# gillet-thomas/NeuroViT

Hardware: AMD Instinct MI355X
Metric: fMRI volumes/sec (fwd+bwd) ViT3D 128^3 p16 d768 L12 [timed step = fwd+bwd+AdamW update] (higher is better)
Workload: dtype bf16; 1 GPU; ViT3D-base 128^3 patch 16, train step (fwd+bwd+AdamW), batch 4/GPU, dropout 0; global_batch=4, parallelism=dp1, grad_buckets=7, grad_allreduce=none (1 GPU)

## Files before the change

### include/neurovit_hip.h

```cpp
#ifndef NEUROVIT_HIP_H
#define NEUROVIT_HIP_H

#ifdef __cplusplus
extern "C" {
#endif

#define NV_OK 0
#define NV_ERR_ARG (-1)
#define NV_ERR_HIP (-2)
#define NV_ERR_ARCH (-3)

int nv_version(void);
int nv_arch_ok(void);
const char* nv_last_error(void);

#define NV_OPERAND_BF16 0
#define NV_OPERAND_FP16 1
int nv_set_operand_format(int fmt);
int nv_operand_format(void);

int nv_prof_enable(int on);
int nv_prof_summary(int kind, double* ms, double* work, long* count);
int nv_prof_summary_bytes(int kind, double* bytes);

// ... 42 lines not shown
  int keep_grads;
  float* params; float* grads; float* adam_m; float* adam_v; void* params16;
} nv_adamw_arena;
int nv_gemm_bf16_grouped_adamw(int count, const nv_gemm_problem* problems, const nv_adamw_arena* opt, void* stream);
int nv_adamw_ranges(const nv_adamw_arena* opt, const long* begins, const long* lens, int count, void* stream);

int nv_gemm_set_tile(int bm, int bn);

int nv_gemm_lnfold_supported(int M, int N, int K);
long nv_ln_fold_stats_floats(int M, int d);
int nv_ln_fold_weight(const float* W, long ldw, int N, int K, const float* gamma, const float* beta, const float* bias, void* Wg16, long ldg,
                      float* colsum, float* fbias, void* stream);
int nv_gemm_resid_ln(int M, int N, int K, const void* A, long lda, const void* W, long ldw, const float* bias, const float* resid, long ldr, float* out,
                     long ldo, void* out16, long ldo16, float* stats, void* stream);
int nv_gemm_lnfold(int gelu, int M, int N, int K, const void* X16, long ldx, const void* Wg16, long ldw, const float* stats, const float* colsum,
                   const float* fbias, float eps, void* out16, long ldo, void* stream);

int nv_skinny_nt(int epi, int R, int N, int K, const void* A, long lda, const void* W, long ldw, const float* bias, const float* resid,
                 long ldr, void* out, long ldo, void* u_out, long ldu, unsigned long drop_seed, float drop_p, void* stream);
int nv_skinny_nn(int epi, int R, int N, int K, const void* A, long lda, const void* W, long ldw, const void* u, long ldu, void* out, long ldo,
                 float* dcol, int accumulate, unsigned long drop_seed, float drop_p, void* stream);
int nv_skinny_nn_sparse(int R, int N, int K, const void* A, long lda, const void* W, long ldw, void* out, long total_rows, int keep_every,
                        void* stream);

int nv_ln_fwd(const float* x, long ldx, int M, int d, const float* gamma, const float* beta, float eps, void* y, long ldy,
              float* mean, float* rstd, void* stream);
long nv_ln_bwd_workspace_bytes(int M, int d);
int nv_ln_bwd(const float* dy, long lddy, const float* x, long ldx, const float* mean, const float* rstd, const float* gamma,
              int M, int d, const float* g_in, float* g_out, long ldg, void* g16, long ldg16, float* dgamma, float* dbeta,
              float* dcolsum, int accumulate, void* workspace, long ws_bytes, unsigned long drop_seed, float drop_p,
              void* stream, void* reduce_stream);
#define NV_LN_NO_REDUCE ((void*)(-1L))
int nv_ln_bwd_reduce(const void* workspace, int M, int d, float* dgamma, float* dbeta, float* dcolsum, int accumulate, void* stream);

typedef struct nv_reduce_job {
  const float* partials;
  int rows, width, nseg;
  float* out[3];
  int accumulate;
} nv_reduce_job;
int nv_reduce_multi(const nv_reduce_job* jobs, int count, void* stream);
int nv_ln_bwd_partial_rows(int M);

long nv_zscore_crop_workspace_bytes(int B);
int nv_volume_sigma(const void* raw, int dtype, const long* strides5, int B, const int* crop8, float eps, float* sigma, float* mean,
                    void* workspace, long ws_bytes, void* stream);
// ... 353 lines not shown
```

### neurovit_amd/_cabi.py

```python
from __future__ import annotations

import ctypes
import os
import re
from typing import Dict, List, Tuple

_HERE = os.path.dirname(os.path.abspath(__file__))
HEADER = os.path.join(os.path.dirname(_HERE), "include", "neurovit_hip.h")
LIB_PATH = os.environ.get("NEUROVIT_HIP_LIB") or os.path.join(_HERE, "lib", "libneurovit_hip.so")

_SCALARS = {"int": ctypes.c_int, "long": ctypes.c_long, "float": ctypes.c_float, "double": ctypes.c_double}


class VitConfig(ctypes.Structure):
    _fields_ = [("image_size", ctypes.c_int), ("image_patch_size", ctypes.c_int), ("frames", ctypes.c_int),
                ("frame_patch_size", ctypes.c_int), ("channels", ctypes.c_int), ("num_classes", ctypes.c_int),
                ("dim", ctypes.c_int), ("depth", ctypes.c_int), ("heads", ctypes.c_int), ("dim_head", ctypes.c_int),
                ("mlp_dim", ctypes.c_int), ("ln_eps", ctypes.c_float), ("pool_mean", ctypes.c_int),
                ("image_width", ctypes.c_int), ("patch_width", ctypes.c_int),
                ("no_proj_dropout", ctypes.c_int)]


class VitInput(ctypes.Structure):
    _fields_ = [("vol_sigma", ctypes.c_void_p), ("time_points", ctypes.c_int), ("rows_form", ctypes.c_int), ("attn_export", ctypes.c_void_p)]
# ... 85 lines not shown
        if self._dll is None:
            if not os.path.exists(LIB_PATH):
                raise RuntimeError(
                    f"neurovit_amd: {LIB_PATH} not found - build it with `python -c 'import __graft_entry__ as g; g.build()'` "
                    "(or `make -C neurovit_amd/csrc`). There is no CPU / PyTorch fallback for this path.")
            dll = ctypes.CDLL(LIB_PATH)
            for name, (restype, argtypes) in self.protos.items():
                fn = getattr(dll, name)
                fn.restype, fn.argtypes = restype, argtypes
            got = dll.nv_abi_version()
            if got != ABI_VERSION:
                raise RuntimeError(f"neurovit_amd: {LIB_PATH} has ABI revision {got}, this binding expects {ABI_VERSION} - rebuild the library "
                                   "(make -C neurovit_amd/csrc); see INTEGRATION.md 'ABI revisions'")
            if os.environ.get("NEUROVIT_ATTN_MODE"):
                dll.nv_attn_set_mode(int(os.environ["NEUROVIT_ATTN_MODE"]))
            if os.environ.get("NEUROVIT_ADAMW_WGS"):
                dll.nv_gemm_set_tile(12, int(os.environ["NEUROVIT_ADAMW_WGS"]))
            if os.environ.get("NEUROVIT_HEAD_STEP"):
                dll.nv_vit_set_head_step(int(os.environ["NEUROVIT_HEAD_STEP"]))
            if os.environ.get("NEUROVIT_WGRAD_WGS"):
                dll.nv_gemm_set_tile(14, int(os.environ["NEUROVIT_WGRAD_WGS"]))
            if os.environ.get("NEUROVIT_PATCH_MODE"):
                dll.nv_patch_set_mode(int(os.environ["NEUROVIT_PATCH_MODE"]))
            if os.environ.get("NEUROVIT_ADAMW_CAP"):
                dll.nv_gemm_set_tile(13, int(os.environ["NEUROVIT_ADAMW_CAP"]))
            self._dll = dll
        return self._dll

    def __getattr__(self, name):
        return getattr(self.load(), name)


lib = _Lib()


OPERAND_FORMATS = {"bf16": 0, "fp16": 1}
_operand_format = "bf16"


def set_operand_format(fmt: str) -> None:
    global _operand_format
    if fmt != _operand_format:
        if fmt not in OPERAND_FORMATS:
            raise ValueError(f"neurovit_amd: operand format must be 'bf16' or 'fp16', got {fmt!r}")
        check(lib.nv_set_operand_format(OPERAND_FORMATS[fmt]), "nv_set_operand_format")
        _operand_format = fmt
# ... 23 lines not shown
```

### neurovit_amd/csrc/engine.hip

```cpp
#include <stdlib.h>
#include <string.h>

#include <unordered_map>
#include <utility>
#include <vector>

#include "../../include/neurovit_hip.h"

#include "common.h"

namespace {

inline long align_up(long v, long a) { return (v + a - 1) / a * a; }

struct Dims {
  int B, N, n, P, Ppad, d, inner, m, L, C, heads, dh, M, T;
  int gf, gh, gw;
  int pool_mean;
};

static int g_cls_tail = 1;
extern "C" int nv_vit_set_cls_tail(int on) { g_cls_tail = on ? 1 : 0; return 0; }
static int g_head_step = 1;
extern "C" int nv_vit_set_head_step(int on) { g_head_step = on ? 1 : 0; return 0; }
// ... 591 lines not shown
    RUN(nv_attn_fwd(ws + w.qkv, 3 * D.inner, B, D.n, D.heads, D.dh, scale, ws + w.ao, D.inner, (float*)(ws + w.lse), site_seed(drop_seed, 4 * l + 0), drop_p, stream));
    if (tail && l == D.L - 1) {
      RUN(cls_rows_block16(D, q, w, l, p, p16, ws, eps, xin, x1, x2, st2, ws + w.u, drop_seed, drop_p, proj_drop_p(cfg, drop_p), stream));
      xin = x2;
      continue;
    }
    RUN(nv_gemm_bf16(0, 4, M, d, D.inner, ws + w.ao, D.inner, p16 + q.wo, D.inner, x1, d, p + q.bo, xin, d, nullptr, 0, 0, 1.f, site_seed(drop_seed, 4 * l + 1), proj_drop_p(cfg, drop_p), stream));
    RUN(nv_ln_fwd_f8_train(x1, d, M, d, p + q.n2g, p + q.n2b, eps, s_xn2, x8, d, ws + w.xn2, d, st2, st2 + M, stream));
    RUN(nv_gemm_f8_gelu_train(M, D.m, d, x8, d, p8 + q.w1, d, cs + 3L * D.inner, p + q.b1, s_h, h8, D.m, ws + w.h, D.m, ws + w.u, D.m,
                              site_seed(drop_seed, 4 * l + 2), drop_p, stream));
    RUN(nv_gemm_f8_resid_drop(M, d, D.m, h8, D.m, p8 + q.w2, D.m, x2, d, cs + 3L * D.inner + D.m, p + q.b2, x1, d, site_seed(drop_seed, 4 * l + 3), drop_p, stream));
    xin = x2;
  }
  return pool_head(D, T, p, eps, xin, ws, W.xm, W.xh, W.hst, logits, stream);
}

namespace {

struct BwdCall {
  const float* video; const long* strides5; const float* params; const void* params16; void* workspace; long ws_bytes; const float* dlogits;
  float* grads; void* grads16;
  int accumulate, first_stage, last_stage; float drop_p, emb_drop_p; unsigned long drop_seed; void* stream; void* aux_stream; int join_aux, rows_form;
  const nv_adamw_arena* fuse; int fuse_mode;
  const nv_vit_backward_opts* opts;
  const nv_vit_attn_grad_export* attn_grad;
};

struct BwdLayer { int l; bool tail; int Mr; long rs; };

struct Bwd {
  const nv_vit_config* cfg; const BwdCall& c; const Dims& D; const ParamTab& T; const WS& W;
  char* ws; const float* p; const r16* p16; float* g;
  bool wg, tail_fwd;
  int M, d, acc, du_tile_rows;
  float scale;
  hipStream_t S, A;
  float* GR(long off) const { return c.grads ? c.grads + off : nullptr; }
  void* M16(long off) const { return c.grads16 ? (void*)((r16*)c.grads16 + off) : nullptr; }
  float* dxn1(int l) const { return (float*)(ws + (l == D.L - 1 ? W.hookg : W.dxn)); }

  int bwd_head() const {
    const float* xlast = (float*)(ws + W.layer[D.L - 1].x2);
    return nv_head_bwd(c.dlogits, D.B, D.C, p + T.hw, D.pool_mean ? (const float*)(ws + W.xm) : xlast, D.pool_mean ? (long)d : (long)D.n * d,
                       (float*)(ws + W.hst), (float*)(ws + W.xh), p + T.hg, d, D.n, g, d, ws + W.scratch(D.L - 1).g16, d,
                       GR(T.hg), GR(T.hb), GR(T.hw), GR(T.hbias), GR(T.layer[D.L - 1].b2), acc, ws + W.sc[0].red, W.red_bytes,
                       site_seed(c.drop_seed, 4 * (D.L - 1) + 3), c.drop_p, D.pool_mean, S);
  }

  int bwd_ffn(const BwdLayer& R) const {
// ... 67 lines not shown
    }
    RUN(nv_reduce_multi(jobs, nj, A));
    nv_gemm_problem pr[4];
    pr[0] = {d, D.m, Mr, g16, d * rs, ws + w.h, D.m * rs, GR(q.w2), D.m, acc, M16(q.w2), D.m};
    pr[1] = {D.m, d, Mr, du, D.m * rs, ws + w.xn2, d * rs, GR(q.w1), d, acc, M16(q.w1), d};
    pr[2] = {d, D.inner, Mr, g16b, d * rs, ws + w.ao, D.inner * rs, GR(q.wo), D.inner, acc, M16(q.wo), D.inner};
    pr[3] = {3 * D.inner, d, M, dqkv, 3 * D.inner, ws + w.xn1, d, GR(q.wqkv), d, acc, M16(q.wqkv), d};
    if (c.fuse && c.fuse_mode != 3) return nv_gemm_bf16_grouped_adamw(4, pr, c.fuse, A);
    return nv_gemm_bf16_grouped(2, 1, 4, pr, A);
  }

  int bwd_embed_tokens() const {
    float* est = (float*)(ws + W.est);
    return nv_embed_finish_bwd(g, d, (float*)(ws + W.t), d, est, est + D.T, p + T.pe_g2, D.B, D.N, d, (float*)(ws + W.dt), d, ws + W.dt16, d, GR(T.pe_g2),
                               GR(T.pe_b2), GR(T.pe_bias), GR(T.pos), GR(T.cls), acc, ws + W.sc[1].red, W.red_bytes, site_seed(c.drop_seed, 4 * D.L), c.emb_drop_p, S);
  }

  int bwd_embed() const {
    float* pst = (float*)(ws + W.pst);
    float* const dvideo = c.opts ? c.opts->dvideo : nullptr;
    const void* wpe = (D.P != D.Ppad) ? (const void*)(ws + W.wpe16) : (const void*)(p16 + T.pe_w);
    void* redA = ws + (A != S ? W.sc[0].red2 : W.sc[0].red);
    const long redA_bytes = A != S ? W.red2_bytes : W.red_bytes;
    RUN(nv_gemm_bf16(1, 1, D.T, D.Ppad, d, ws + W.dt16, d, wpe, D.Ppad, ws + W.dxp, D.Ppad, nullptr, nullptr, 0, nullptr, 0, 0, 1.f, 0, 0.f, A));
    if (dvideo)
      RUN(nv_patch_ln_dx(c.video, c.strides5, D.B, cfg->channels, cfg->frames, cfg->image_size, img_w(cfg), cfg->image_patch_size, pat_w(cfg), cfg->frame_patch_size,
                         (const float*)(ws + W.dxp), D.Ppad, pst, pst + D.T, p + T.pe_g, dvideo, c.opts->dvideo_strides5, A));
    if (!wg) return NV_OK;
    RUN(nv_patch_ln_bwd(c.video, c.strides5, D.B, cfg->channels, cfg->frames, cfg->image_size, img_w(cfg), cfg->image_patch_size,
                        pat_w(cfg), cfg->frame_patch_size, (float*)(ws + W.dxp), D.Ppad, pst, pst + D.T, GR(T.pe_g), GR(T.pe_b), acc, redA, redA_bytes, A));
    if (D.P != D.Ppad) {
      RUN(nv_gemm_bf16(2, 1, d, D.Ppad, D.T, ws + W.dt16, d, ws + W.xp, D.Ppad, ws + W.dwpe, D.Ppad, nullptr, nullptr, 0, nullptr, 0, 0, 1.f, 0, 0.f, S));
      return nv_copy_2d_f32((float*)(ws + W.dwpe), D.Ppad, d, D.P, GR(T.pe_w), D.P, acc, S);
    }
    return nv_gemm_bf16(2, 1, d, D.P, D.T, ws + W.dt16, d, ws + W.xp, D.Ppad, GR(T.pe_w), D.P, nullptr, nullptr, 0, M16(T.pe_w), D.P, acc, 1.f, 0, 0.f, S);
  }
};

}

static int backward_impl(const Layout& Y, const nv_vit_config* cfg, const BwdCall& c) {
  const Dims& D = Y.D; const WS& W = Y.W;
  const nv_adamw_arena* fuse = c.fuse; const nv_vit_backward_opts* opts = c.opts;
  NV_CHECK_ARG(!fuse || (!c.accumulate && !c.grads16 && fuse->grads == c.grads && c.first_stage <= 1 && c.last_stage == D.L + 1),
               "nv_vit_backward: the optimizer update during the backward pass needs accumulate = 0, no bf16 mirror, its own gradient arena and every stage in one call");
  const bool wg = !opts || opts->weight_grads;
  NV_CHECK_ARG(!fuse || !opts, "nv_vit_backward: the optimizer update during the backward pass takes no input gradient / data-only options");
  NV_CHECK_ARG(!fuse || !c.attn_grad, "nv_vit_backward: the optimizer update during the backward pass exports no attention gradients");
  NV_CHECK_ARG(!opts || !opts->dvideo || opts->dvideo_strides5, "nv_vit_backward_ex: dvideo needs dvideo_strides5");
  NV_CHECK_ARG(wg || (!c.grads && !c.grads16), "nv_vit_backward_ex: the data-only backward (weight_grads = 0) writes no gradient arena - pass grads = grads16 = NULL");
  NV_CHECK_ARG(c.video && c.strides5 && c.params && c.params16 && c.workspace && c.dlogits && (c.grads || !wg), "nv_vit_backward: null pointer");
  NV_CHECK_ARG(c.ws_bytes >= W.total, "nv_vit_backward: workspace too small (%ld < %ld) - forward must run with training=1", c.ws_bytes, W.total);
  NV_CHECK_ARG(nv_aligned16(c.grads) && nv_aligned16(c.grads16), "nv_vit_backward: grads / grads16 must be 16-byte aligned");
  NV_CHECK_ARG(c.first_stage >= 0 && c.last_stage <= D.L + 1 && c.first_stage <= c.last_stage, "nv_vit_backward_stages: bad stage range [%d, %d]", c.first_stage, c.last_stage);
  hipStream_t S = (hipStream_t)c.stream;
  hipStream_t A = (c.aux_stream && wg) ? (hipStream_t)c.aux_stream : S;
  const bool forked = (A != S);
  char* ws = (char*)c.workspace;
// ... 240 lines not shown
  const Dims& D = Y.D; const ParamTab& T = Y.T; const WS& W = Y.W;
  RUN(forward_in_impl(Y, cfg, B, video, shape5, strides5, in, params, params16, workspace, ws_bytes, 1, drop_p, emb_drop_p, drop_seed, logits, stream, head_fused));
  if (head_fused) {
    char* ws = (char*)workspace;
    const int Ll = D.L - 1;
    RUN(nv_head_step_soft((const float*)(ws + W.layer[Ll].x2), (long)D.n * D.d, B, D.d, params + T.hg, params + T.hb, cfg->ln_eps, params + T.hw, params + T.hbias, D.C,
                          labels, lscale, hp->loss_scale_state, lo, (float*)(ws + W.xh), (float*)(ws + W.hst), logits, loss, dlogits, D.n, (float*)(ws + W.g), D.d,
                          ws + W.scratch(Ll).g16, D.d, grads + T.hg, grads + T.hb, grads + T.hw, grads + T.hbias, grads + T.layer[Ll].b2,
                          hp->accumulate ? 1 : 0, ws + W.sc[0].red, W.red_bytes, site_seed(drop_seed, 4 * Ll + 3), drop_p, stream));
  } else {
    RUN(nv_ce_loss_soft(logits, labels, B, cfg->num_classes, lscale, hp->loss_scale_state, lo, loss, dlogits, stream));
  }
  nv_adamw_arena opt;
  opt.struct_size = (int)sizeof(opt); opt.step = hp->step; opt.lr = hp->lr; opt.beta1 = hp->beta1; opt.beta2 = hp->beta2; opt.eps = hp->eps;
  opt.weight_decay = hp->weight_decay; opt.grad_scale = hp->grad_scale / lscale; opt.keep_grads = hp->fuse_update == 2;
  opt.params = params; opt.grads = grads; opt.adam_m = adam_m; opt.adam_v = adam_v; opt.params16 = params16;
  BwdCall bc{};
  bc.video = video; bc.strides5 = strides5; bc.params = params; bc.params16 = params16; bc.workspace = workspace; bc.ws_bytes = ws_bytes;
  bc.dlogits = dlogits; bc.grads = grads; bc.accumulate = hp->accumulate ? 1 : 0; bc.drop_p = drop_p; bc.emb_drop_p = emb_drop_p; bc.drop_seed = drop_seed;
  bc.stream = stream; bc.aux_stream = aux_stream; bc.join_aux = 1; bc.rows_form = in ? in->rows_form : 0;
  if (dp && hp->update) return dp_backward_update(Y, cfg, bc, params, params16, adam_m, adam_v, hp, dp, head_fused, lscale);
  bc.first_stage = head_fused ? 1 : 0; bc.last_stage = cfg->depth + 1;
  bc.fuse = fused ? &opt : nullptr; bc.fuse_mode = hp->fuse_update;
  RUN(backward_impl(Y, cfg, bc));
  if (hp->update && !fused) {
    RUN(final_update(hp, params, params16, grads, nullptr, adam_m, adam_v, T.total, hp->grad_scale / lscale, stream));
  } else if (fused) {
    std::vector<long> begins, lens;
    long cur = 0;
    auto skip = [&](long off, long numel) { if (off > cur) { begins.push_back(cur); lens.push_back(off - cur); } cur = align_up(off + numel, 8); };
    for (int l = 0; l < D.L; ++l) {
      const LinearW lw = linear_weights(D, T.layer[l]);
      for (int i = 0; i < 4; ++i) skip(lw.off[i], lw.numel[i]);
    }
    if (T.total > cur) { begins.push_back(cur); lens.push_back(T.total - cur); }
    RUN(nv_adamw_ranges(&opt, begins.data(), lens.data(), (int)begins.size(), stream));
  }
  return NV_OK;
}
```

### neurovit_amd/csrc/norm.hip

```cpp
#include "common.h"

#define WAVES_PER_BLOCK 4

#include <type_traits>
template <typename OT>
__device__ __forceinline__ void store4(OT* p, const f32x4& o) {
  if constexpr (std::is_same<OT, float>::value) *reinterpret_cast<f32x4*>(p) = o;
  else *reinterpret_cast<r16x4*>(p) = cvt4<OT>(o[0], o[1], o[2], o[3]);
}
__device__ __forceinline__ r16 cvt1_rt(float v, int fp16) { return fp16 ? cvt1<fp16_t>(v) : cvt1<bf16_t>(v); }

template <int NV>
__device__ __forceinline__ void row_load(const float* row, int d, int lane, f32x4 (&x)[NV]) {
#pragma unroll
  for (int v = 0; v < NV; ++v) {
    const int c = (lane + 64 * v) * 4;
    x[v] = (c < d) ? *reinterpret_cast<const f32x4*>(row + c) : f32x4{0.f, 0.f, 0.f, 0.f};
  }
}
template <int NV>
__device__ __forceinline__ void row_stats(const f32x4 (&x)[NV], int d, int lane, float eps, float& mean, float& rstd) {
  float s = 0.f;
#pragma unroll
  for (int v = 0; v < NV; ++v) s += (x[v][0] + x[v][1]) + (x[v][2] + x[v][3]);
// ... 902 lines not shown
                                   unsigned long drop_seed, float drop_p, void* stream) {
  const DropCfg drop = make_drop(drop_seed, drop_p);
  NV_CHECK_ARG(B > 0 && N > 0 && (d % 4) == 0 && d <= 2048, "nv_embed_finish_fwd: d=%d must be a multiple of 4 and <= 2048", d);
  NV_CHECK_ARG((ldt % 4) == 0 && (ldx % 4) == 0, "nv_embed_finish_fwd: leading dims must be multiples of 4");
  const int rows = B * (N + 1);
  const dim3 grid((rows + WAVES_PER_BLOCK - 1) / WAVES_PER_BLOCK), block(256);
  hipStream_t s = (hipStream_t)stream;
  if (d <= 1024) hipLaunchKernelGGL(embed_finish_fwd_kernel<4>, grid, block, 0, s, t, ldt, B, N, d, gamma, beta, eps, pos, cls, x, ldx, mean, rstd, drop);
  else hipLaunchKernelGGL(embed_finish_fwd_kernel<8>, grid, block, 0, s, t, ldt, B, N, d, gamma, beta, eps, pos, cls, x, ldx, mean, rstd, drop);
  NV_CHECK_LAUNCH("nv_embed_finish_fwd");
  return NV_OK;
}

__global__ void batch_sum_kernel(const float* __restrict__ g, long ldg, int B, int n, int d, float* dpos, float* dcls, int accumulate) {
  const long idx = (long)blockIdx.x * blockDim.x + threadIdx.x;
  if (idx >= (long)n * d) return;
  const int i = (int)(idx / d), c = (int)(idx - (long)i * d);
  float s = 0.f;
  for (int b = 0; b < B; ++b) s += g[((long)b * n + i) * ldg + c];
  if (dpos) dpos[idx] = accumulate ? dpos[idx] + s : s;
  if (i == 0 && dcls) dcls[c] = accumulate ? dcls[c] + s : s;
}

__global__ void apply_drop_kernel(float* __restrict__ g, long count, DropCfg drop) {
  const long i = ((long)blockIdx.x * blockDim.x + threadIdx.x) * 4;
  if (i >= count) return;
  f32x4 v = *reinterpret_cast<f32x4*>(g + i);
  v *= drop_factor4(drop, (unsigned long long)i);
  *reinterpret_cast<f32x4*>(g + i) = v;
}

extern "C" long nv_embed_finish_bwd_workspace_bytes(int B, int N, int d) { return nv_ln_bwd_workspace_bytes(B * N, d); }

extern "C" int nv_embed_finish_bwd(const float* g, long ldg, const float* t, long ldt, const float* mean, const float* rstd,
                                   const float* gamma, int B, int N, int d, float* dt, long lddt, void* dt16, long lddt16,
                                   float* dgamma, float* dbeta, float* dbias_pe, float* dpos, float* dcls, int accumulate,
                                   void* workspace, long ws_bytes, unsigned long drop_seed, float drop_p, void* stream) {
  hipStream_t s = (hipStream_t)stream;
  const DropCfg drop = make_drop(drop_seed, drop_p);
  if (drop.thresh) {
    NV_CHECK_ARG(ldg == d, "nv_embed_finish_bwd: dropout needs a dense g");
    const long count = (long)B * (N + 1) * d;
    hipLaunchKernelGGL(apply_drop_kernel, dim3((unsigned)((count / 4 + 255) / 256)), dim3(256), 0, s, (float*)g, count, drop);
    NV_CHECK_LAUNCH("nv_embed_finish_bwd/drop");
  }
  NV_CHECK_ARG(B > 0 && N > 0 && (d % 4) == 0 && d <= 2048, "nv_embed_finish_bwd: bad dims");
  const int n = N + 1;
  const long need = nv_embed_finish_bwd_workspace_bytes(B, N, d);
  NV_CHECK_ARG(ws_bytes >= need, "nv_embed_finish_bwd: workspace too small");
  const bool params_out = dgamma || dbeta || dbias_pe || dpos || dcls;
  NV_CHECK_ARG(!params_out || (dgamma && dbeta && dbias_pe && dpos && dcls), "nv_embed_finish_bwd: the parameter gradients are all given or all NULL");
  {
    const int rc = ln_bwd_launch(g + ldg, ldg, t, ldt, mean, rstd, gamma, B * N, d, nullptr, dt, lddt, dt16, lddt16, dgamma, dbeta, dbias_pe,
                                 accumulate, workspace, ws_bytes, 0, 0.f, stream, params_out ? nullptr : NV_LN_NO_REDUCE, N, 1);
    if (rc) return rc;
  }
  if (!params_out) return NV_OK;
  const long tot = (long)n * d;
  hipLaunchKernelGGL(batch_sum_kernel, dim3((unsigned)((tot + 255) / 256)), dim3(256), 0, s, g, ldg, B, n, d, dpos, dcls, accumulate);
  NV_CHECK_LAUNCH("nv_embed_finish_bwd/batch_sum");
  return NV_OK;
}

__device__ __forceinline__ void head_fwd_row(int b, float* sh, const float* __restrict__ x, long row_stride, int d, const float* __restrict__ gamma,
                                             const float* __restrict__ beta, float eps, const float* __restrict__ Wt,
                                             const float* __restrict__ bias, int C, float* __restrict__ xh_out,
                                             float* __restrict__ stats_out, float* __restrict__ logits) {
  float* xs = sh;
  float* scratch = sh + d;
  const int tid = threadIdx.x, lane = tid & 63, wid = tid >> 6;
  const float* row = x + (long)b * row_stride;
  float s = 0.f;
  for (int c = tid; c < d; c += 256) { xs[c] = row[c]; s += xs[c]; }
  s = wave_sum(s);
  if (lane == 0) scratch[wid] = s;
  __syncthreads();
  const float mean = ((scratch[0] + scratch[1]) + (scratch[2] + scratch[3])) / (float)d;
  float q = 0.f;
  for (int c = tid; c < d; c += 256) { const float t = xs[c] - mean; q += t * t; }
  q = wave_sum(q);
  if (lane == 0) scratch[4 + wid] = q;
  __syncthreads();
// ... 336 lines not shown
```

### neurovit_amd/csrc/skinny.hip

```cpp
#include "common.h"

namespace {

constexpr int SK_R = 4;

enum { SK_NT_RESID = 0, SK_NT_GELU = 1 };
enum { SK_NN_DGELU = 0, SK_NN_F32 = 1, SK_NN_BF16 = 2 };

template <int EPI, typename T>
__global__ __launch_bounds__(256) void skinny_nt_kernel(const r16* __restrict__ A, long lda, int R, const r16* __restrict__ W, long ldw, int N, int K,
                                                        const float* __restrict__ bias, const float* __restrict__ resid, long ldr,
                                                        void* __restrict__ out, long ldo, r16* __restrict__ u_out, long ldu, DropCfg drop) {
  const int lane = threadIdx.x & 63, n = blockIdx.x * 4 + (threadIdx.x >> 6);
  const int r0 = blockIdx.y * SK_R, rows = (R - r0 < SK_R) ? R - r0 : SK_R;
  if (n >= N) return;
  float acc[SK_R];
#pragma unroll
  for (int r = 0; r < SK_R; ++r) acc[r] = 0.f;
  const r16* w = W + (long)n * ldw;
  for (int k = lane * 8; k < K; k += 4 * 512) {
    r16x8 wq[4], aq[4][SK_R];
#pragma unroll
    for (int q = 0; q < 4; ++q) {
      const int kq = k + 512 * q;
// ... 44 lines not shown
template <int EPI, typename T>
__global__ __launch_bounds__(1024) void skinny_nn_kernel(const r16* __restrict__ A, long lda, int R, const r16* __restrict__ W, long ldw, int N, int K,
                                                         const r16* __restrict__ u, long ldu, void* __restrict__ out, long ldo,
                                                         float* __restrict__ dcol, int accumulate, long fill_rows, int keep_every, DropCfg drop) {
  extern __shared__ __attribute__((aligned(16))) float sk_lds[];
  if (blockIdx.z == 1) {
    zero_rows_except(reinterpret_cast<char*>(out), fill_rows, (long)N * 2, keep_every, blockIdx.y * gridDim.x + blockIdx.x, gridDim.x * gridDim.y);
    return;
  }
  float (*part)[NN_KK][SK_R][NN_COLS] = reinterpret_cast<float (*)[NN_KK][SK_R][NN_COLS]>(sk_lds);
  float (*red)[SK_R][NN_COLS] = reinterpret_cast<float (*)[SK_R][NN_COLS]>(sk_lds + 16 * NN_KK * SK_R * NN_COLS);
  const int tid = threadIdx.x, lane = tid & 63, wv = tid >> 6, ng = lane & (NN_COLS / 8 - 1), kk = lane / (NN_COLS / 8);
  const int n0 = blockIdx.x * NN_COLS, nc = n0 + ng * 8;
  const int r0 = blockIdx.y * SK_R, rows = (R - r0 < SK_R) ? R - r0 : SK_R;
  float acc[SK_R][8];
#pragma unroll
  for (int r = 0; r < SK_R; ++r)
#pragma unroll
    for (int e = 0; e < 8; ++e) acc[r][e] = 0.f;
  if (nc < N) {
    constexpr int STEP = 16 * NN_KK;
    for (int k = wv * NN_KK + kk; k < K; k += 4 * STEP) {
      r16x8 wq[4];
      float aq[4][SK_R];
#pragma unroll
      for (int q = 0; q < 4; ++q) {
        const int kq = k + STEP * q;
        if (kq < K) {
          wq[q] = *reinterpret_cast<const r16x8*>(W + (long)kq * ldw + nc);
#pragma unroll
          for (int r = 0; r < SK_R; ++r)
            if (r < rows) aq[q][r] = dec1<T>(A[(long)(r0 + r) * lda + kq]);
        }
      }
#pragma unroll
      for (int q = 0; q < 4; ++q) {
        if (k + STEP * q < K) {
#pragma unroll
          for (int r = 0; r < SK_R; ++r) {
            if (r < rows) {
#pragma unroll
              for (int e = 0; e < 8; ++e) acc[r][e] = __builtin_fmaf(aq[q][r], dec1<T>(wq[q][e]), acc[r][e]);
            }
          }
        }
      }
    }
  }
#pragma unroll
  for (int r = 0; r < SK_R; ++r) {
    *reinterpret_cast<f32x4*>(&part[wv][kk][r][ng * 8]) = f32x4{acc[r][0], acc[r][1], acc[r][2], acc[r][3]};
    *reinterpret_cast<f32x4*>(&part[wv][kk][r][ng * 8 + 4]) = f32x4{acc[r][4], acc[r][5], acc[r][6], acc[r][7]};
  }
  __syncthreads();
  {
    const int w = tid / (SK_R * NN_COLS), rc = tid % (SK_R * NN_COLS);
    float v = 0.f;
#pragma unroll
    for (int q = 0; q < NN_KK; ++q) v += part[w][q][rc / NN_COLS][rc % NN_COLS];
    red[w][rc / NN_COLS][rc % NN_COLS] = v;
  }
  __syncthreads();
  const int c = tid % NN_COLS, r = tid / NN_COLS;
  float stored = 0.f;
  const bool live = r < rows && n0 + c < N;
// ... 8 lines not shown
      const r16 o = cvt1<T>(v * keep * gelu_grad_f(dec1<T>(u[row * ldu + n])));
      ((r16*)out)[row * ldo + n] = o;
      stored = dec1<T>(o);
    } else if constexpr (EPI == SK_NN_F32) {
      ((float*)out)[row * ldo + n] = v;
    } else {
      ((r16*)out)[row * ldo + n] = cvt1<T>(v);
    }
  }
  if constexpr (EPI == SK_NN_DGELU) {
    if (dcol) {
      __syncthreads();
      if (r < SK_R) red[0][r][c] = live ? stored : 0.f;
      __syncthreads();
      if (r == 0 && n0 + c < N) {
        float s = 0.f;
#pragma unroll
        for (int q = 0; q < SK_R; ++q) s += red[0][q][c];
        dcol[n0 + c] = (accumulate ? dcol[n0 + c] : 0.f) + s;
      }
    }
  }
}

constexpr int NN_LDS = (16 * NN_KK * SK_R * NN_COLS + 16 * SK_R * NN_COLS) * (int)sizeof(float);
template <typename T>
void nn_attrs_fmt() {
  (void)hipFuncSetAttribute(reinterpret_cast<const void*>(skinny_nn_kernel<SK_NN_DGELU, T>), hipFuncAttributeMaxDynamicSharedMemorySize, NN_LDS);
  (void)hipFuncSetAttribute(reinterpret_cast<const void*>(skinny_nn_kernel<SK_NN_F32, T>), hipFuncAttributeMaxDynamicSharedMemorySize, NN_LDS);
  (void)hipFuncSetAttribute(reinterpret_cast<const void*>(skinny_nn_kernel<SK_NN_BF16, T>), hipFuncAttributeMaxDynamicSharedMemorySize, NN_LDS);
}
void nn_attrs() {
  static bool attr = false;
  if (attr) return;
  nn_attrs_fmt<bf16_t>(); nn_attrs_fmt<fp16_t>();
  attr = true;
}

}

extern "C" int nv_skinny_nt(int epi, int R, int N, int K, const void* A, long lda, const void* W, long ldw, const float* bias, const float* resid,
                            long ldr, void* out, long ldo, void* u_out, long ldu, unsigned long drop_seed, float drop_p, void* stream) {
  NV_CHECK_ARG(drop_p == 0.f || (ldo % N) == 0, "nv_skinny_nt: with dropout `out` must be a row-strided view of a dense [M, N] tensor (ldo a multiple of N)");
  const DropCfg drop = make_drop(drop_seed, drop_p);
  NV_CHECK_ARG(R > 0 && N > 0 && K > 0 && (K % 8) == 0 && (lda % 8) == 0 && (ldw % 8) == 0 && A && W && bias && out && nv_aligned16(A) && nv_aligned16(W),
               "nv_skinny_nt: K, lda, ldw must be multiples of 8, operands 16-byte aligned");
  NV_CHECK_ARG(epi == SK_NT_GELU || (epi == SK_NT_RESID && resid), "nv_skinny_nt: epilogue 0 needs resid; epilogues are 0 (bias + residual, f32) and 1 (bias + GELU, bf16)");
  const dim3 grid((N + 3) / 4, (R + SK_R - 1) / SK_R), block(256);
  hipStream_t s = (hipStream_t)stream;
  NV_DISPATCH_OPERAND(T,
    if (epi == SK_NT_RESID)
      hipLaunchKernelGGL((skinny_nt_kernel<SK_NT_RESID, T>), grid, block, 0, s, (const r16*)A, lda, R, (const r16*)W, ldw, N, K, bias, resid, ldr, out, ldo, (r16*)nullptr, 0L, drop);
    else
      hipLaunchKernelGGL((skinny_nt_kernel<SK_NT_GELU, T>), grid, block, 0, s, (const r16*)A, lda, R, (const r16*)W, ldw, N, K, bias, resid, ldr, out, ldo, (r16*)u_out, ldu, drop));
  NV_CHECK_LAUNCH("nv_skinny_nt");
  return NV_OK;
}

extern "C" int nv_skinny_nn(int epi, int R, int N, int K, const void* A, long lda, const void* W, long ldw, const void* u, long ldu, void* out, long ldo,
                            float* dcol, int accumulate, unsigned long drop_seed, float drop_p, void* stream) {
  NV_CHECK_ARG(drop_p == 0.f || (epi == SK_NN_DGELU && (ldo % N) == 0), "nv_skinny_nn: dropout only with epilogue 0, `out` a row-strided view of a dense [M, N] tensor");
  const DropCfg drop = make_drop(drop_seed, drop_p);
  NV_CHECK_ARG(R > 0 && N > 0 && K > 0 && (N % 8) == 0 && (ldw % 8) == 0 && A && W && out && nv_aligned16(W), "nv_skinny_nn: N, ldw must be multiples of 8, W 16-byte aligned");
  NV_CHECK_ARG(epi >= 0 && epi <= 2 && (epi != SK_NN_DGELU || u) && (!dcol || (epi == SK_NN_DGELU && R <= SK_R)), "nv_skinny_nn: epilogue 0 needs u; column sums only with epilogue 0 and R <= 4");
  const dim3 grid((N + NN_COLS - 1) / NN_COLS, (R + SK_R - 1) / SK_R), block(1024);
  hipStream_t s = (hipStream_t)stream;
  nn_attrs();
#define SK_NN(E) hipLaunchKernelGGL((skinny_nn_kernel<E, T>), grid, block, NN_LDS, s, (const r16*)A, lda, R, (const r16*)W, ldw, N, K, (const r16*)u, ldu, out, ldo, dcol, accumulate, 0L, 0, drop)
  NV_DISPATCH_OPERAND(T, if (epi == SK_NN_DGELU) SK_NN(SK_NN_DGELU); else if (epi == SK_NN_F32) SK_NN(SK_NN_F32); else SK_NN(SK_NN_BF16));
#undef SK_NN
  NV_CHECK_LAUNCH("nv_skinny_nn");
  return NV_OK;
}

extern "C" int nv_skinny_nn_sparse(int R, int N, int K, const void* A, long lda, const void* W, long ldw, void* out, long total_rows, int keep_every,
                                   void* stream) {
  NV_CHECK_ARG(R > 0 && N > 0 && K > 0 && (N % 8) == 0 && (ldw % 8) == 0 && A && W && out && nv_aligned16(W) && nv_aligned16(out) && keep_every >= 1 &&
                   (long)(R - 1) * keep_every < total_rows && (long)R * keep_every >= total_rows,
               "nv_skinny_nn_sparse: N, ldw multiples of 8; W, out 16-byte aligned; R = ceil(total_rows / keep_every) (every kept row is computed: the fill skips them all)");
  const dim3 grid((N + NN_COLS - 1) / NN_COLS, (R + SK_R - 1) / SK_R, 2), block(1024);
  nn_attrs();
  NV_DISPATCH_OPERAND(T, hipLaunchKernelGGL((skinny_nn_kernel<SK_NN_BF16, T>), grid, block, NN_LDS, (hipStream_t)stream, (const r16*)A, lda, R, (const r16*)W, ldw, N, K,
                                            (const r16*)nullptr, 0L, out, (long)N * keep_every, (float*)nullptr, 0, total_rows, keep_every, make_drop(0, 0.f)));
  NV_CHECK_LAUNCH("nv_skinny_nn_sparse");
  return NV_OK;
}
```

Measured before the change: 1191 volumes/s.

## Add split-K skinny NN kernel, vectorized batch sum, and overlap rest-param AdamW

Adds a split-K variant of the skinny NN GEMM. When K exceeds 2048 by default, it spreads the reduction over many workgroups and merges the partial sums through a global scratch buffer with an atomic last-block counter, so that only a few row tiles no longer underfill the GPU. It also vectorizes the position/cls gradient batch-sum to float4 with one block per token. Separately, when fused updates are on and an aux stream exists, it splits the remaining-parameter AdamW update across two streams and moves the patch-embed dx GEMM to the main stream. The existing skinny NN inner loop now loads A values as bf16 and clamps out-of-range k instead of branching. The split-K path relies on device-global counters and scratch, which adds a cross-block synchronisation risk.

```diff
diff --git a/include/neurovit_hip.h b/include/neurovit_hip.h
--- a/include/neurovit_hip.h
+++ b/include/neurovit_hip.h
@@ -88,6 +88,7 @@
                  float* dcol, int accumulate, unsigned long drop_seed, float drop_p, void* stream);
 int nv_skinny_nn_sparse(int R, int N, int K, const void* A, long lda, const void* W, long ldw, void* out, long total_rows, int keep_every,
                         void* stream);
+int nv_skinny_set_mode(int mode);
 
 int nv_ln_fwd(const float* x, long ldx, int M, int d, const float* gamma, const float* beta, float eps, void* y, long ldy,
               float* mean, float* rstd, void* stream);
diff --git a/neurovit_amd/_cabi.py b/neurovit_amd/_cabi.py
--- a/neurovit_amd/_cabi.py
+++ b/neurovit_amd/_cabi.py
@@ -131,6 +131,8 @@
                 dll.nv_gemm_set_tile(14, int(os.environ["NEUROVIT_WGRAD_WGS"]))
             if os.environ.get("NEUROVIT_PATCH_MODE"):
                 dll.nv_patch_set_mode(int(os.environ["NEUROVIT_PATCH_MODE"]))
+            if os.environ.get("NEUROVIT_SKINNY_MODE"):
+                dll.nv_skinny_set_mode(int(os.environ["NEUROVIT_SKINNY_MODE"]))
             if os.environ.get("NEUROVIT_ADAMW_CAP"):
                 dll.nv_gemm_set_tile(13, int(os.environ["NEUROVIT_ADAMW_CAP"]))
             self._dll = dll
diff --git a/neurovit_amd/csrc/engine.hip b/neurovit_amd/csrc/engine.hip
--- a/neurovit_amd/csrc/engine.hip
+++ b/neurovit_amd/csrc/engine.hip
@@ -637,9 +637,33 @@
   float* grads; void* grads16;
   int accumulate, first_stage, last_stage; float drop_p, emb_drop_p; unsigned long drop_seed; void* stream; void* aux_stream; int join_aux, rows_form;
   const nv_adamw_arena* fuse; int fuse_mode;
+  bool fuse_rest;
   const nv_vit_backward_opts* opts;
   const nv_vit_attn_grad_export* attn_grad;
 };
+
+void rest_update_ranges(const Dims& D, const ParamTab& T, int part, std::vector<long>& begins, std::vector<long>& lens) {
+  const long main_iv[3][2] = {{T.pos, T.pe_g}, {T.pe_w, T.layer[0].n1g}, {T.layer[D.L - 1].b2, T.total}};
+  auto push = [&](long b, long e) { if (e > b) { begins.push_back(b); lens.push_back(e - b); } };
+  auto emit = [&](long b, long e) {
+    if (part == 0) return push(b, e);
+    for (int i = 0; i < 3 && b < e; ++i) {
+      const long lo = main_iv[i][0], hi = main_iv[i][1];
+      if (hi <= b || lo >= e) continue;
+      if (lo > b) { if (part == 2) push(b, lo); b = lo; }
+      const long m = hi < e ? hi : e;
+      if (part == 1) push(b, m);
+      b = m;
+    }
+    if (part == 2) push(b, e);
+  };
+  long cur = 0;
+  for (int l = 0; l < D.L; ++l) {
+    const LinearW lw = linear_weights(D, T.layer[l]);
+    for (int i = 0; i < 4; ++i) { emit(cur, lw.off[i]); cur = align_up(lw.off[i] + lw.numel[i], 8); }
+  }
+  emit(cur, T.total);
+}
 
 struct BwdLayer { int l; bool tail; int Mr; long rs; };
 
@@ -753,7 +777,9 @@
     const void* wpe = (D.P != D.Ppad) ? (const void*)(ws + W.wpe16) : (const void*)(p16 + T.pe_w);
     void* redA = ws + (A != S ? W.sc[0].red2 : W.sc[0].red);
     const long redA_bytes = A != S ? W.red2_bytes : W.red_bytes;
-    RUN(nv_gemm_bf16(1, 1, D.T, D.Ppad, d, ws + W.dt16, d, wpe, D.Ppad, ws + W.dxp, D.Ppad, nullptr, nullptr, 0, nullptr, 0, 0, 1.f, 0, 0.f, A));
+    const hipStream_t Q = c.fuse_rest ? S : A;
+    RUN(nv_gemm_bf16(1, 1, D.T, D.Ppad, d, ws + W.dt16, d, wpe, D.Ppad, ws + W.dxp, D.Ppad, nullptr, nullptr, 0, nullptr, 0, 0, 1.f, 0, 0.f, Q));
+    if (c.fuse_rest) RUN(stream_sync(S, A));
     if (dvideo)
       RUN(nv_patch_ln_dx(c.video, c.strides5, D.B, cfg->channels, cfg->frames, cfg->image_size, img_w(cfg), cfg->image_patch_size, pat_w(cfg), cfg->frame_patch_size,
                          (const float*)(ws + W.dxp), D.Ppad, pst, pst + D.T, p + T.pe_g, dvideo, c.opts->dvideo_strides5, A));
@@ -762,9 +788,17 @@
                         pat_w(cfg), cfg->frame_patch_size, (float*)(ws + W.dxp), D.Ppad, pst, pst + D.T, GR(T.pe_g), GR(T.pe_b), acc, redA, redA_bytes, A));
     if (D.P != D.Ppad) {
       RUN(nv_gemm_bf16(2, 1, d, D.Ppad, D.T, ws + W.dt16, d, ws + W.xp, D.Ppad, ws + W.dwpe, D.Ppad, nullptr, nullptr, 0, nullptr, 0, 0, 1.f, 0, 0.f, S));
-      return nv_copy_2d_f32((float*)(ws + W.dwpe), D.Ppad, d, D.P, GR(T.pe_w), D.P, acc, S);
-    }
-    return nv_gemm_bf16(2, 1, d, D.P, D.T, ws + W.dt16, d, ws + W.xp, D.Ppad, GR(T.pe_w), D.P, nullptr, nullptr, 0, M16(T.pe_w), D.P, acc, 1.f, 0, 0.f, S);
+      RUN(nv_copy_2d_f32((float*)(ws + W.dwpe), D.Ppad, d, D.P, GR(T.pe_w), D.P, acc, S));
+    } else {
+      RUN(nv_gemm_bf16(2, 1, d, D.P, D.T, ws + W.dt16, d, ws + W.xp, D.Ppad, GR(T.pe_w), D.P, nullptr, nullptr, 0, M16(T.pe_w), D.P, acc, 1.f, 0, 0.f, S));
+    }
+    if (!c.fuse_rest) return NV_OK;
+    std::vector<long> b, n;
+    rest_update_ranges(D, T, 1, b, n);
+    RUN(nv_adamw_ranges(c.fuse, b.data(), n.data(), (int)b.size(), S));
+    b.clear(); n.clear();
+    rest_update_ranges(D, T, 2, b, n);
+    return nv_adamw_ranges(c.fuse, b.data(), n.data(), (int)b.size(), A);
   }
 };
 
@@ -1051,18 +1085,13 @@
   if (dp && hp->update) return dp_backward_update(Y, cfg, bc, params, params16, adam_m, adam_v, hp, dp, head_fused, lscale);
   bc.first_stage = head_fused ? 1 : 0; bc.last_stage = cfg->depth + 1;
   bc.fuse = fused ? &opt : nullptr; bc.fuse_mode = hp->fuse_update;
+  bc.fuse_rest = fused && aux_stream && aux_stream != stream;
   RUN(backward_impl(Y, cfg, bc));
   if (hp->update && !fused) {
     RUN(final_update(hp, params, params16, grads, nullptr, adam_m, adam_v, T.total, hp->grad_scale / lscale, stream));
-  } else if (fused) {
+  } else if (fused && !bc.fuse_rest) {
     std::vector<long> begins, lens;
-    long cur = 0;
-    auto skip = [&](long off, long numel) { if (off > cur) { begins.push_back(cur); lens.push_back(off - cur); } cur = align_up(off + numel, 8); };
-    for (int l = 0; l < D.L; ++l) {
-      const LinearW lw = linear_weights(D, T.layer[l]);
-      for (int i = 0; i < 4; ++i) skip(lw.off[i], lw.numel[i]);
-    }
-    if (T.total > cur) { begins.push_back(cur); lens.push_back(T.total - cur); }
+    rest_update_ranges(D, T, 0, begins, lens);
     RUN(nv_adamw_ranges(&opt, begins.data(), lens.data(), (int)begins.size(), stream));
   }
   return NV_OK;
diff --git a/neurovit_amd/csrc/norm.hip b/neurovit_amd/csrc/norm.hip
--- a/neurovit_amd/csrc/norm.hip
+++ b/neurovit_amd/csrc/norm.hip
@@ -948,6 +948,32 @@
   if (i == 0 && dcls) dcls[c] = accumulate ? dcls[c] + s : s;
 }
 
+__global__ __launch_bounds__(256) void batch_sum4_kernel(const float* __restrict__ g, long ldg, int B, int n, int d, float* dpos, float* dcls, int accumulate) {
+  const int i = blockIdx.x;
+  for (int c = threadIdx.x * 4; c < d; c += 256 * 4) {
+    const float* src = g + (long)i * ldg + c;
+    const long bstep = (long)n * ldg;
+    f32x4 s = {0.f, 0.f, 0.f, 0.f};
+    int b = 0;
+    for (; b + 4 <= B; b += 4) {
+      f32x4 v[4];
+#pragma unroll
+      for (int q = 0; q < 4; ++q) v[q] = *reinterpret_cast<const f32x4*>(src + (b + q) * bstep);
+#pragma unroll
+      for (int q = 0; q < 4; ++q) s += v[q];
+    }
+    for (; b < B; ++b) s += *reinterpret_cast<const f32x4*>(src + b * bstep);
+    if (dpos) {
+      f32x4* o = reinterpret_cast<f32x4*>(dpos + (long)i * d + c);
+      *o = accumulate ? *o + s : s;
+    }
+    if (i == 0 && dcls) {
+      f32x4* o = reinterpret_cast<f32x4*>(dcls + c);
+      *o = accumulate ? *o + s : s;
+    }
+  }
+}
+
 __global__ void apply_drop_kernel(float* __restrict__ g, long count, DropCfg drop) {
   const long i = ((long)blockIdx.x * blockDim.x + threadIdx.x) * 4;
   if (i >= count) return;
@@ -983,7 +1009,10 @@
   }
   if (!params_out) return NV_OK;
   const long tot = (long)n * d;
-  hipLaunchKernelGGL(batch_sum_kernel, dim3((unsigned)((tot + 255) / 256)), dim3(256), 0, s, g, ldg, B, n, d, dpos, dcls, accumulate);
+  if ((ldg % 4) == 0 && nv_aligned16(g) && nv_aligned16(dpos) && nv_aligned16(dcls))
+    hipLaunchKernelGGL(batch_sum4_kernel, dim3((unsigned)n), dim3(256), 0, s, g, ldg, B, n, d, dpos, dcls, accumulate);
+  else
+    hipLaunchKernelGGL(batch_sum_kernel, dim3((unsigned)((tot + 255) / 256)), dim3(256), 0, s, g, ldg, B, n, d, dpos, dcls, accumulate);
   NV_CHECK_LAUNCH("nv_embed_finish_bwd/batch_sum");
   return NV_OK;
 }
diff --git a/neurovit_amd/csrc/skinny.hip b/neurovit_amd/csrc/skinny.hip
--- a/neurovit_amd/csrc/skinny.hip
+++ b/neurovit_amd/csrc/skinny.hip
@@ -90,16 +90,13 @@
     constexpr int STEP = 16 * NN_KK;
     for (int k = wv * NN_KK + kk; k < K; k += 4 * STEP) {
       r16x8 wq[4];
-      float aq[4][SK_R];
+      r16 aq[4][SK_R];
 #pragma unroll
       for (int q = 0; q < 4; ++q) {
-        const int kq = k + STEP * q;
-        if (kq < K) {
-          wq[q] = *reinterpret_cast<const r16x8*>(W + (long)kq * ldw + nc);
-#pragma unroll
-          for (int r = 0; r < SK_R; ++r)
-            if (r < rows) aq[q][r] = dec1<T>(A[(long)(r0 + r) * lda + kq]);
-        }
+        const int kq = k + STEP * q, kc = kq < K ? kq : K - 1;
+        wq[q] = *reinterpret_cast<const r16x8*>(W + (long)kc * ldw + nc);
+#pragma unroll
+        for (int r = 0; r < SK_R; ++r) aq[q][r] = A[(long)(r0 + (r < rows ? r : rows - 1)) * lda + kc];
       }
 #pragma unroll
       for (int q = 0; q < 4; ++q) {
@@ -107,8 +104,9 @@
 #pragma unroll
           for (int r = 0; r < SK_R; ++r) {
             if (r < rows) {
-#pragma unroll
-              for (int e = 0; e < 8; ++e) acc[r][e] = __builtin_fmaf(aq[q][r], dec1<T>(wq[q][e]), acc[r][e]);
+              const float a = dec1<T>(aq[q][r]);
+#pragma unroll
+              for (int e = 0; e < 8; ++e) acc[r][e] = __builtin_fmaf(a, dec1<T>(wq[q][e]), acc[r][e]);
             }
           }
         }
@@ -163,6 +161,146 @@
     }
   }
 }
+
+constexpr int NS_COLS = 64;
+constexpr int NS_KK = 32;
+constexpr int NS_BATCH = 6;
+constexpr int NS_PAD = 4;
+constexpr int NS_MIN_CHUNK = 64;
+constexpr int NS_TARGET_WGS = 256;
+constexpr int NS_SLAB = SK_R * NS_COLS;
+constexpr long NS_SCRATCH_FLOATS = 1L << 20;
+constexpr int NS_COUNTERS = 4096;
+__device__ float ns_scratch[NS_SCRATCH_FLOATS];
+__device__ unsigned ns_count[NS_COUNTERS];
+
+template <int EPI, typename T>
+__global__ __launch_bounds__(256) void skinny_nn_split_kernel(const r16* __restrict__ A, long lda, int R, const r16* __restrict__ W, long ldw, int N, int K,
+                                                              const r16* __restrict__ u, long ldu, void* __restrict__ out, long ldo,
+                                                              float* __restrict__ dcol, int accumulate, int ksplit, int chunk, long fill_rows, int keep_every,
+                                                              DropCfg drop) {
+  __shared__ __attribute__((aligned(16))) float part[NS_KK][NS_SLAB + NS_PAD];
+  __shared__ int last;
+  const int tid = threadIdx.x;
+  if ((int)blockIdx.z >= ksplit) {
+    zero_rows_except(reinterpret_cast<char*>(out), fill_rows, (long)N * 2, keep_every, ((blockIdx.z - ksplit) * gridDim.y + blockIdx.y) * gridDim.x + blockIdx.x,
+                     (gridDim.z - ksplit) * gridDim.y * gridDim.x);
+    return;
+  }
+  const int ng = tid & 7, kk = tid >> 3;
+  const int n0 = blockIdx.x * NS_COLS, nc = n0 + ng * 8;
+  const int r0 = blockIdx.y * SK_R, rows = (R - r0 < SK_R) ? R - r0 : SK_R;
+  const int kz = blockIdx.z, k_lo = kz * chunk, k_hi = (k_lo + chunk < K) ? k_lo + chunk : K;
+  float acc[SK_R][8];
+#pragma unroll
+  for (int r = 0; r < SK_R; ++r)
+#pragma unroll
+    for (int e = 0; e < 8; ++e) acc[r][e] = 0.f;
+  if (nc < N) {
+    for (int kb = k_lo; kb < k_hi; kb += NS_BATCH * NS_KK) {
+      r16x8 wq[NS_BATCH];
+      r16 aq[NS_BATCH][SK_R];
+      bool in[NS_BATCH];
+#pragma unroll
+      for (int q = 0; q < NS_BATCH; ++q) {
+        const int kq = kb + NS_KK * q + kk;
+        in[q] = kq < k_hi;
+        const int kc = in[q] ? kq : k_hi - 1;
+        wq[q] = *reinterpret_cast<const r16x8*>(W + (long)kc * ldw + nc);
+#pragma unroll
+        for (int r = 0; r < SK_R; ++r) aq[q][r] = A[(long)(r0 + (r < rows ? r : rows - 1)) * lda + kc];
+      }
+#pragma unroll
+      for (int q = 0; q < NS_BATCH; ++q) {
+        const r16x8 wz = in[q] ? wq[q] : r16x8{0, 0, 0, 0, 0, 0, 0, 0};
+#pragma unroll
+        for (int r = 0; r < SK_R; ++r) {
+          const float a = in[q] ? dec1<T>(aq[q][r]) : 0.f;
+#pragma unroll
+          for (int e = 0; e < 8; ++e) acc[r][e] = __builtin_fmaf(a, dec1<T>(wz[e]), acc[r][e]);
+        }
+      }
+    }
+  }
+#pragma unroll
+  for (int r = 0; r < SK_R; ++r) {
+    *reinterpret_cast<f32x4*>(&part[kk][r * NS_COLS + ng * 8]) = f32x4{acc[r][0], acc[r][1], acc[r][2], acc[r][3]};
+    *reinterpret_cast<f32x4*>(&part[kk][r * NS_COLS + ng * 8 + 4]) = f32x4{acc[r][4], acc[r][5], acc[r][6], acc[r][7]};
+  }
+  __syncthreads();
+  float v = 0.f;
+#pragma unroll
+  for (int q = 0; q < NS_KK; ++q) v += part[q][tid];
+  if (ksplit > 1) {
+    const int group = blockIdx.y * gridDim.x + blockIdx.x;
+    float* slab = ns_scratch + (long)group * ksplit * NS_SLAB;
+    __hip_atomic_store(slab + kz * NS_SLAB + tid, v, __ATOMIC_RELAXED, __HIP_MEMORY_SCOPE_AGENT);
+    asm volatile("s_waitcnt vmcnt(0)" ::: "memory");
+    __syncthreads();
+    if (tid == 0) {
+      const unsigned before = __hip_atomic_fetch_add(&ns_count[group], 1u, __ATOMIC_RELAXED, __HIP_MEMORY_SCOPE_AGENT);
+      last = before == (unsigned)ksplit - 1;
+      if (last) {
+        __builtin_amdgcn_fence(__ATOMIC_ACQUIRE, "agent");
+        asm volatile("s_waitcnt vmcnt(0)" ::: "memory");
+        __hip_atomic_store(&ns_count[group], 0u, __ATOMIC_RELAXED, __HIP_MEMORY_SCOPE_AGENT);
+      }
+    }
+    __syncthreads();
+    if (!last) return;
+    v = 0.f;
+#pragma unroll 4
+    for (int p = 0; p < ksplit; ++p) v += __hip_atomic_load(slab + p * NS_SLAB + tid, __ATOMIC_RELAXED, __HIP_MEMORY_SCOPE_AGENT);
+  }
+  const int c = tid % NS_COLS, r = tid / NS_COLS;
+  float stored = 0.f;
+  const bool live = r < rows && n0 + c < N;
+  if (live) {
+    const long row = r0 + r;
+    const int n = n0 + c;
+    if constexpr (EPI == SK_NN_DGELU) {
+      const float keep = drop.thresh ? drop_factor(drop, (unsigned long long)(row * ldo + n)) : 1.f;
+      const r16 o = cvt1<T>(v * keep * gelu_grad_f(dec1<T>(u[row * ldu + n])));
+      ((r16*)out)[row * ldo + n] = o;
+      stored = dec1<T>(o);
+    } else if constexpr (EPI == SK_NN_F32) {
+      ((float*)out)[row * ldo + n] = v;
+    } else {
+      ((r16*)out)[row * ldo + n] = cvt1<T>(v);
+    }
+  }
+  if constexpr (EPI == SK_NN_DGELU) {
+    if (dcol) {
+      __syncthreads();
+      part[0][tid] = live ? stored : 0.f;
+      __syncthreads();
+      if (r == 0 && n0 + c < N) {
+        float s = 0.f;
+#pragma unroll
+        for (int q = 0; q < SK_R; ++q) s += part[0][q * NS_COLS + c];
+        dcol[n0 + c] = (accumulate ? dcol[n0 + c] : 0.f) + s;
+      }
+    }
+  }
+}
+
+struct NnSplit { int groups, slices, ksplit, chunk; };
+NnSplit nn_split(int R, int N, int K) {
+  NnSplit s;
+  s.groups = (N + NS_COLS - 1) / NS_COLS;
+  s.slices = (R + SK_R - 1) / SK_R;
+  const long cells = (long)s.groups * s.slices;
+  long want = (NS_TARGET_WGS + cells - 1) / cells;
+  if (want > K / NS_MIN_CHUNK) want = K / NS_MIN_CHUNK;
+  if (want < 1 || cells > NS_COUNTERS) want = 1;
+  s.chunk = (int)(((K + want - 1) / want + NS_KK - 1) / NS_KK * NS_KK);
+  s.ksplit = (K + s.chunk - 1) / s.chunk;
+  if (s.ksplit > 1 && cells * s.ksplit * NS_SLAB > NS_SCRATCH_FLOATS) { s.ksplit = 1; s.chunk = (K + NS_KK - 1) / NS_KK * NS_KK; }
+  return s;
+}
+
+int g_skinny_mode = 0;
+inline bool nn_split_form(int K) { return g_skinny_mode == 2 || (g_skinny_mode == 0 && K > 2048); }
 
 constexpr int NN_LDS = (16 * NN_KK * SK_R * NN_COLS + 16 * SK_R * NN_COLS) * (int)sizeof(float);
 template <typename T>
@@ -198,14 +336,25 @@
   return NV_OK;
 }
 
+extern "C" int nv_skinny_set_mode(int mode) { g_skinny_mode = (mode == 1 || mode == 2) ? mode : 0; return 0; }
+
 extern "C" int nv_skinny_nn(int epi, int R, int N, int K, const void* A, long lda, const void* W, long ldw, const void* u, long ldu, void* out, long ldo,
                             float* dcol, int accumulate, unsigned long drop_seed, float drop_p, void* stream) {
   NV_CHECK_ARG(drop_p == 0.f || (epi == SK_NN_DGELU && (ldo % N) == 0), "nv_skinny_nn: dropout only with epilogue 0, `out` a row-strided view of a dense [M, N] tensor");
   const DropCfg drop = make_drop(drop_seed, drop_p);
   NV_CHECK_ARG(R > 0 && N > 0 && K > 0 && (N % 8) == 0 && (ldw % 8) == 0 && A && W && out && nv_aligned16(W), "nv_skinny_nn: N, ldw must be multiples of 8, W 16-byte aligned");
   NV_CHECK_ARG(epi >= 0 && epi <= 2 && (epi != SK_NN_DGELU || u) && (!dcol || (epi == SK_NN_DGELU && R <= SK_R)), "nv_skinny_nn: epilogue 0 needs u; column sums only with epilogue 0 and R <= 4");
+  hipStream_t s = (hipStream_t)stream;
+  if (nn_split_form(K)) {
+    const NnSplit sp = nn_split(R, N, K);
+    const dim3 grid(sp.groups, sp.slices, sp.ksplit), block(256);
+#define SK_NS(E) hipLaunchKernelGGL((skinny_nn_split_kernel<E, T>), grid, block, 0, s, (const r16*)A, lda, R, (const r16*)W, ldw, N, K, (const r16*)u, ldu, out, ldo, dcol, accumulate, sp.ksplit, sp.chunk, 0L, 0, drop)
+    NV_DISPATCH_OPERAND(T, if (epi == SK_NN_DGELU) SK_NS(SK_NN_DGELU); else if (epi == SK_NN_F32) SK_NS(SK_NN_F32); else SK_NS(SK_NN_BF16));
+#undef SK_NS
+    NV_CHECK_LAUNCH("nv_skinny_nn");
+    return NV_OK;
+  }
   const dim3 grid((N + NN_COLS - 1) / NN_COLS, (R + SK_R - 1) / SK_R), block(1024);
-  hipStream_t s = (hipStream_t)stream;
   nn_attrs();
 #define SK_NN(E) hipLaunchKernelGGL((skinny_nn_kernel<E, T>), grid, block, NN_LDS, s, (const r16*)A, lda, R, (const r16*)W, ldw, N, K, (const r16*)u, ldu, out, ldo, dcol, accumulate, 0L, 0, drop)
   NV_DISPATCH_OPERAND(T, if (epi == SK_NN_DGELU) SK_NN(SK_NN_DGELU); else if (epi == SK_NN_F32) SK_NN(SK_NN_F32); else SK_NN(SK_NN_BF16));
@@ -219,6 +368,16 @@
   NV_CHECK_ARG(R > 0 && N > 0 && K > 0 && (N % 8) == 0 && (ldw % 8) == 0 && A && W && out && nv_aligned16(W) && nv_aligned16(out) && keep_every >= 1 &&
                    (long)(R - 1) * keep_every < total_rows && (long)R * keep_every >= total_rows,
                "nv_skinny_nn_sparse: N, ldw multiples of 8; W, out 16-byte aligned; R = ceil(total_rows / keep_every) (every kept row is computed: the fill skips them all)");
+  if (nn_split_form(K)) {
+    const NnSplit sp = nn_split(R, N, K);
+    const int fill = (NS_TARGET_WGS + sp.groups * sp.slices - 1) / (sp.groups * sp.slices);
+    const dim3 grid(sp.groups, sp.slices, sp.ksplit + fill), block(256);
+    NV_DISPATCH_OPERAND(T, hipLaunchKernelGGL((skinny_nn_split_kernel<SK_NN_BF16, T>), grid, block, 0, (hipStream_t)stream, (const r16*)A, lda, R, (const r16*)W, ldw, N, K,
+                                              (const r16*)nullptr, 0L, out, (long)N * keep_every, (float*)nullptr, 0, sp.ksplit, sp.chunk, total_rows, keep_every,
+                                              make_drop(0, 0.f)));
+    NV_CHECK_LAUNCH("nv_skinny_nn_sparse");
+    return NV_OK;
+  }
   const dim3 grid((N + NN_COLS - 1) / NN_COLS, (R + SK_R - 1) / SK_R, 2), block(1024);
   nn_attrs();
   NV_DISPATCH_OPERAND(T, hipLaunchKernelGGL((skinny_nn_kernel<SK_NN_BF16, T>), grid, block, NN_LDS, (hipStream_t)stream, (const r16*)A, lda, R, (const r16*)W, ldw, N, K,
```

After: 1191 volumes/s. Within noise of the previous version (-0.0%).
